# patrikhuber/superviseddescent

Measured on NVIDIA H100. Metric: faces/sec RCR 22-landmark detect, higher is better.
Workload: dtype f32

## Files before the change

superviseddescent_b200/csrc/sd_hog.cu:

```cuda
#include "sd_internal.cuh"
#include "sd_hog_common.cuh"

#include <cmath>
#include <cuda_pipeline.h>

namespace {

constexpr int kHogThreads = 256;

struct HogArgs {
    const uint8_t* images;
    int width, height, row_stride;
    long long image_stride;
    int image_count;
    const int* image_index;
    const sd_roi* roi;
    const sd_frame* frames;
    uint8_t* roi_miss;
    const float* x;
    long long ldx;
    int N, L;
    int variant, nc, cs, K, fs, dd;
    const int* half;
    HogOrient orient;
    const int* rtab;
    const float* btab;
    int tma_count;
    float* A;
    long long ld;
    int* geometry;
    uint8_t* patches;
    int8_t* bins;
    int* status;
};

__global__ void hog_geometry_kernel(const float* __restrict__ x, long long ldx, int N, int L, const sd_eyes_dev eyes, float rel,
                                    int fixed_half, int fs, int* __restrict__ half_out, int* __restrict__ rtab, int* __restrict__ status,
                                    uint8_t* __restrict__ face_flag)
{
    const int i = blockIdx.x;
    if (i >= N) return;
    __shared__ int s_half;
    if (threadIdx.x == 0) {
        bool degenerate;
        const int half = sd_patch_half(x + (long long)i * ldx, L, eyes, rel, fixed_half, &degenerate);
        if (degenerate) {
            atomicOr(status, 1);
            if (face_flag) face_flag[i] = 1;
        }
        half_out[i] = half;
        s_half = half;
    }
    __syncthreads();
    const int P = 2 * s_half;
    int* rt = rtab + (long long)i * 5 * fs;
    for (int t = threadIdx.x; t < fs; t += blockDim.x) {
        const HogResizeTap r = hog_resize_tap(t, fs, P);
        rt[t] = r.sx;
        rt[fs + t] = r.xw;
        rt[2 * fs + t] = r.y0;
        rt[3 * fs + t] = r.y1;
        rt[4 * fs + t] = r.yw;
    }
}

__global__ void hog_bintab_kernel(int fs, int nc, int cs, int pw, float* __restrict__ btab)
{
    __shared__ int s_sbin[256];
    for (int t = threadIdx.x; t < fs; t += blockDim.x) {
        int b;
        float w1, w2;
        hog_spatial_weight(t, cs, &b, &w1, &w2);
        s_sbin[t] = b;
        if (t >= 1 && t <= fs - 2)
            for (int c = 0; c < nc; ++c) btab[c * pw + t - 1] = (b == c) ? w1 : ((b == c - 1) ? w2 : 0.f);
        else if (t == fs - 1 && pw > fs - 2)
            for (int c = 0; c < nc; ++c) btab[c * pw + pw - 1] = 0.f;
    }
    __syncthreads();
    int* lohi = reinterpret_cast<int*>(btab + nc * pw);
    for (int c = threadIdx.x; c < nc; c += blockDim.x) {
        int lo = fs, hi = -1;
        for (int t = 1; t <= fs - 2; ++t) {
            const int b = s_sbin[t];
            if (b == c || b == c - 1) { if (t < lo) lo = t; hi = t; }
        }
        lohi[c] = lo;
        lohi[nc + c] = hi;
    }
}

__device__ __forceinline__ int byte_of(unsigned lo, unsigned hi, int n) { return (int)(((n < 4 ? lo : hi) >> (8 * (n & 3))) & 0xffu); }

struct HogSmem {
    int patch, bin, r1, tab, xa, wcell, lo, hi, vote, mbar, stage_end, total;
    int pp;
    int pb, pm;
    int pw;
    int tpad;
};

__host__ __device__ inline int align_up(int v, int a) { return (v + a - 1) / a * a; }

__host__ __device__ inline HogSmem hog_smem_layout(int fs, int nc, int K)
{
    HogSmem s;
    s.pp = align_up(fs, 4);
    s.pm = align_up(fs - 2, 4) + 1;
    s.pb = s.pm - 1;
    if ((s.pb & 7) == 0 && (fs - 2) * (s.pb + 4) <= fs * fs) s.pb += 4;
    int o = 0;
    s.patch = o;
    o = align_up(s.pp * fs, 16);
    s.tab = o;    o += fs * 16;
    s.xa = o;     o += fs * 4;
    s.pw = align_up(fs - 2, 2);
    s.wcell = align_up(o, 8); o = s.wcell + nc * s.pw * 4;
    s.lo = o;     o += nc * 4;
    s.hi = o;     o += nc * 4;
    s.mbar = align_up(o, 8); o = s.mbar + 8;
    o = align_up(o, 128);
    s.bin = o;    o = align_up(o + fs * fs, 16);
    s.r1 = o;     o = align_up(o + fs * fs * 4, 16);
    s.tpad = align_up((fs - 2) * nc, 32);
    s.vote = o;
    o += 2 * K * s.tpad * 4;
    s.stage_end = o;
    s.total = align_up(o + 8, 16);
    return s;
}

constexpr int kTmaClasses = 8;
__host__ __device__ constexpr int hog_tma_box(int c) { return c == 0 ? 32 : c == 1 ? 48 : c == 2 ? 64 : c == 3 ? 80 : c == 4 ? 96 : c == 5 ? 112 : c == 6 ? 128 : 160; }
struct HogMaps { CUtensorMap m[kTmaClasses]; };

template <bool MIR>
__device__ __forceinline__ bool hog_sample_mirrored(const HogArgs& a, int sample)
{
    return MIR && sd_sample_is_mirrored(a.image_index[sample]);
}

template <int KT, int NCT, int CST, int NT, bool MIR>
__global__ void __launch_bounds__(NT, NCT > 0 ? 2048 / NT : 0) hog_patch_kernel(const __grid_constant__ HogArgs a, const __grid_constant__ HogMaps maps)
{
    static_assert(NT % 32 == 0 && NT >= 64, "hog_patch_kernel needs whole warps and at least 64 threads");
    constexpr int kWarps = NT / 32;
    extern __shared__ __align__(128) unsigned char smem[];
    const int K = KT > 0 ? KT : a.K;
    const int nc = NCT > 0 ? NCT : a.nc;
    const int fs = (NCT > 0 && CST > 0) ? NCT * CST : a.fs;
    const int cells = nc * nc;
    const HogSmem lay = hog_smem_layout(fs, nc, K);
    const int pp = lay.pp, pb = lay.pb, pm = lay.pm, pw = lay.pw;
    uint8_t* s_patch = smem + lay.patch;
    int8_t* s_bin = reinterpret_cast<int8_t*>(smem + lay.bin);
    float* s_gmag = reinterpret_cast<float*>(smem + lay.r1);
    int4* s_tab = reinterpret_cast<int4*>(smem + lay.tab);
    short2* s_xa = reinterpret_cast<short2*>(smem + lay.xa);
    float* s_wcell = reinterpret_cast<float*>(smem + lay.wcell);
    int* s_lo = reinterpret_cast<int*>(smem + lay.lo);
    int* s_hi = reinterpret_cast<int*>(smem + lay.hi);
    float* s_T = reinterpret_cast<float*>(smem + lay.vote);
    uint64_t* s_mbar = reinterpret_cast<uint64_t*>(smem + lay.mbar);

    const int tid = threadIdx.x;
    const int lane = tid & 31, warp = tid >> 5;
    const long long patch_id = blockIdx.x;
    const int sample = (int)(patch_id / a.L);
    const int lm = (int)(patch_id - (long long)sample * a.L);

    const float* __restrict__ row = a.x + (long long)sample * a.ldx;
    const int half = __ldg(a.half + sample);
    const int P = 2 * half;
    const int cx = __float2int_rn(row[lm]);
    const int cy = __float2int_rn(row[lm + a.L]);
    int img_idx = a.image_index ? a.image_index[sample] : sample;
    if (MIR) img_idx = sd_sample_frame_of(img_idx);
    if (img_idx < 0 || img_idx >= a.image_count) {
        img_idx = 0;
        if (tid == 0 && a.status) atomicOr(a.status, 2);
    }
    int W = a.width, H = a.height, rs = a.row_stride;
    const uint8_t* __restrict__ img = a.images + (long long)img_idx * a.image_stride;
    if (a.frames) {
        const sd_frame f = a.frames[img_idx];
        W = f.width; H = f.height; rs = f.row_stride;
        img = a.images + f.offset;
    }
    int rx = 0, ry = 0, rw = W, rh = H;
    if (a.roi) {
        const sd_roi r = a.roi[img_idx];
        rx = r.x; ry = r.y; rw = r.w; rh = r.h; rs = r.row_stride;
        img = a.images + r.offset;
    }
    if (tid == 0 && a.geometry) {
        a.geometry[patch_id * 3 + 0] = cx;
        a.geometry[patch_id * 3 + 1] = cy;
        a.geometry[patch_id * 3 + 2] = half;
    }

    const int x0 = sd_window_x0(cx, half, W, hog_sample_mirrored<MIR>(a, sample)), y0 = cy - half;
    uint8_t* s_stage = smem + lay.bin;
    const int stage_cap = lay.stage_end - lay.bin;
    int tma_box = 0;
    const int tma_shift = x0 & 15;
#pragma unroll
    for (int c = kTmaClasses - 1; c >= 0; --c)
        if (c < a.tma_count && hog_tma_box(c) >= P + tma_shift && hog_tma_box(c) * hog_tma_box(c) <= stage_cap) tma_box = hog_tma_box(c);
    if (tma_box > 0 && tid == 0) {
        int cls = 0;
#pragma unroll
        for (int c = 0; c < kTmaClasses; ++c) if (hog_tma_box(c) == tma_box) cls = c;
        hog_tma_load(s_mbar, s_stage, &maps.m[cls], x0 - tma_shift, y0, img_idx, tma_box * tma_box);
    }

    {
        const int* __restrict__ rt = a.rtab + (long long)sample * 5 * fs;
        for (int t = tid; t < fs; t += NT) {
            const int xa = __ldg(rt + fs + t);
            s_xa[t] = *reinterpret_cast<const short2*>(&xa);
            s_tab[t] = make_int4(__ldg(rt + t), __ldg(rt + 2 * fs + t), __ldg(rt + 3 * fs + t), __ldg(rt + 4 * fs + t));
        }
        for (int i = tid; i < nc * pw; i += NT) s_wcell[i] = __ldg(a.btab + i);
        const int* __restrict__ lohi = reinterpret_cast<const int*>(a.btab + nc * pw);
        if (tid < nc) { s_lo[tid] = __ldg(lohi + tid); s_hi[tid] = __ldg(lohi + nc + tid); }
    }
    {
        const bool resident = x0 >= rx && y0 >= ry && x0 + P <= rx + rw && y0 + P <= ry + rh && x0 >= 0 && y0 >= 0 && x0 + P <= W && y0 + P <= H;
        const uintptr_t align_bits = reinterpret_cast<uintptr_t>(img) | (uintptr_t)rs;
        const bool vec16 = !tma_box && resident && (align_bits & 15) == 0;
        const bool words = !tma_box && resident && (align_bits & 3) == 0;
        const int shiftb = tma_box ? tma_shift : (vec16 ? ((x0 - rx) & 15) : (words ? ((x0 - rx) & 3) : 0));
        const int pitch = tma_box ? tma_box : ((P + 15 + 15) & ~15);
        const bool staged = pitch * P <= stage_cap;
        bool miss = false;
        if (staged) {
            if (tma_box) {
            } else if (vec16) {
                const int nvec = (shiftb + P + 15) >> 4;
                const int gs = nvec <= 8 ? 3 : (nvec <= 16 ? 4 : 5);
                const int lv = lane & ((1 << gs) - 1), lr = lane >> gs, rows_per_pass = 32 >> gs;
                const uint8_t* wrow = img + (long long)(y0 - ry) * rs + (x0 - rx - shiftb);
                for (int r = warp * rows_per_pass + lr; r < P; r += kWarps * rows_per_pass)
#pragma unroll 1
                    for (int v = lv; v < nvec; v += (1 << gs))
                        reinterpret_cast<uint4*>(s_stage + r * pitch)[v] = __ldg(reinterpret_cast<const uint4*>(wrow + (long long)r * rs) + v);
            } else if (words) {
                const int nwords = (shiftb + P + 3) >> 2;
                const uint8_t* wrow = img + (long long)(y0 - ry) * rs + (x0 - rx - shiftb);
                for (int r = warp; r < P; r += kWarps) {
                    const uint32_t* src = reinterpret_cast<const uint32_t*>(wrow + (long long)r * rs);
                    uint32_t* dst = reinterpret_cast<uint32_t*>(s_stage + r * pitch);
#pragma unroll 1
                    for (int w = lane; w < nwords; w += 32) dst[w] = __ldg(src + w);
                }
            } else {
                for (int r = warp; r < P; r += kWarps) {
                    const int iy = y0 + r;
                    const bool rowin = (unsigned)iy < (unsigned)H;
                    const bool rowres = iy >= ry && iy < ry + rh;
                    for (int c = lane; c < P; c += 32) {
                        const int ix = x0 + c;
                        int v = 0;
                        if (rowin && (unsigned)ix < (unsigned)W) {
                            if (rowres && ix >= rx && ix < rx + rw) v = __ldg(img + (long long)(iy - ry) * rs + (ix - rx));
                            else miss = true;
                        }
                        s_stage[r * pitch + c] = (uint8_t)v;
                    }
                }
            }
            __syncthreads();
            if (tma_box) hog_tma_wait(s_mbar);
            if (hog_sample_mirrored<MIR>(a, sample)) {
#pragma unroll 1
                for (int r = warp; r < P; r += kWarps) {
                    uint8_t* q = s_stage + r * pitch + shiftb;
#pragma unroll 1
                    for (int c = lane; c < half; c += 32) {
                        const uint8_t u = q[c], v = q[P - 1 - c];
                        q[c] = v;
                        q[P - 1 - c] = u;
                    }
                }
                __syncthreads();
            }
            if (fs <= 64) {
                const int np = (fs + 1) >> 1, groups = NT / np;
                const int j = tid % np, g = tid / np;
                if (g < groups) {
                    const int dxa = 2 * j, dxb = min(dxa + 1, fs - 1);
                    const int sxa = s_tab[dxa].x, sxb = s_tab[dxb].x;
                    const unsigned xa = *reinterpret_cast<const unsigned*>(s_xa + dxa), xb = *reinterpret_cast<const unsigned*>(s_xa + dxb);
                    const int q = (shiftb + sxa) & ~3;
                    const int oa = shiftb + sxa - q, ob = shiftb + sxb - q;
                    uint8_t* out = s_patch + dxa;
                    if (ob <= 6) {
                        const unsigned sa = oa | (oa + 1) << 4, sb = ob | (ob + 1) << 4;
                        const uint8_t* base = s_stage + q;
#pragma unroll 2
                        for (int dy = g; dy < fs; dy += groups) {
                            const int4 yt = s_tab[dy];
                            const unsigned* r0 = reinterpret_cast<const unsigned*>(base + yt.y * pitch);
                            const unsigned* r1 = reinterpret_cast<const unsigned*>(base + yt.z * pitch);
                            const unsigned a0 = r0[0], a1 = r0[1], b0 = r1[0], b1 = r1[1];
                            const int va = hog_resize_out(yt.w, __dp2a_lo(xa, __byte_perm(a0, a1, sa), 0u), __dp2a_lo(xa, __byte_perm(b0, b1, sa), 0u));
                            const int vb = hog_resize_out(yt.w, __dp2a_lo(xb, __byte_perm(a0, a1, sb), 0u), __dp2a_lo(xb, __byte_perm(b0, b1, sb), 0u));
                            *reinterpret_cast<uint16_t*>(out + dy * pp) = (uint16_t)(va | vb << 8);
                        }
                    } else {
                        const int ax = s_xa[dxa].x, bx = s_xa[dxa].y, cx = s_xa[dxb].x, dx = s_xa[dxb].y;
                        const int sxa1 = min(sxa + 1, P - 1), sxb1 = min(sxb + 1, P - 1);
                        const uint8_t* base = s_stage + shiftb;
                        for (int dy = g; dy < fs; dy += groups) {
                            const int4 yt = s_tab[dy];
                            const uint8_t* r0 = base + yt.y * pitch;
                            const uint8_t* r1 = base + yt.z * pitch;
                            const int va = hog_resize_out(yt.w, (int)r0[sxa] * ax + (int)r0[sxa1] * bx, (int)r1[sxa] * ax + (int)r1[sxa1] * bx);
                            const int vb = hog_resize_out(yt.w, (int)r0[sxb] * cx + (int)r0[sxb1] * dx, (int)r1[sxb] * cx + (int)r1[sxb1] * dx);
                            *reinterpret_cast<uint16_t*>(out + dy * pp) = (uint16_t)(va | vb << 8);
                        }
                    }
                }
            } else {
                for (int dy = warp; dy < fs; dy += kWarps) {
                    const int4 yt = s_tab[dy];
                    const uint8_t* r0 = s_stage + yt.y * pitch + shiftb;
                    const uint8_t* r1 = s_stage + yt.z * pitch + shiftb;
                    for (int dx = lane; dx < fs; dx += 32) {
                        const int sx = s_tab[dx].x;
                        const int sx1 = min(sx + 1, P - 1);
                        const short2 xa = s_xa[dx];
                        const int t0 = (int)r0[sx] * xa.x + (int)r0[sx1] * xa.y;
                        const int t1 = (int)r1[sx] * xa.x + (int)r1[sx1] * xa.y;
                        s_patch[dy * pp + dx] = (uint8_t)hog_resize_out(yt.w, t0, t1);
                    }
                }
            }
        } else {
            const bool mirrored = hog_sample_mirrored<MIR>(a, sample);
            __syncthreads();
            for (int dy = warp; dy < fs; dy += kWarps) {
                const int4 yt = s_tab[dy];
                const int iy0 = y0 + yt.y, iy1 = y0 + yt.z;
                for (int dx = lane; dx < fs; dx += 32) {
                    const int sx = s_tab[dx].x;
                    const short2 xa = s_xa[dx];
                    int p[4];
#pragma unroll
                    for (int q = 0; q < 4; ++q) {
                        const int u = sx + (q & 1);
                        const int ix = mirrored ? x0 + P - 1 - u : x0 + u, iy = (q & 2) ? iy1 : iy0;
                        int v = 0;
                        if ((q & 1) && xa.y == 0) { p[q] = 0; continue; }
                        if ((unsigned)ix < (unsigned)W && (unsigned)iy < (unsigned)H) {
                            if (ix >= rx && ix < rx + rw && iy >= ry && iy < ry + rh) v = __ldg(img + (long long)(iy - ry) * rs + (ix - rx));
                            else miss = true;
                        }
                        p[q] = v;
                    }
                    const int t0 = p[0] * xa.x + p[1] * xa.y;
                    const int t1 = p[2] * xa.x + p[3] * xa.y;
                    s_patch[dy * pp + dx] = (uint8_t)hog_resize_out(yt.w, t0, t1);
                }
            }
        }
        if (miss && a.roi_miss) a.roi_miss[img_idx] = 1;
        if (a.patches) {
            __syncthreads();
            for (int i = tid; i < fs * fs; i += NT) {
                const int y = i / fs;
                a.patches[patch_id * fs * fs + i] = s_patch[y * pp + (i - y * fs)];
            }
        }
    }
    __syncthreads();

    {
        const int iw = fs - 2, runs = (iw + 3) >> 2, nitem = iw * runs;
        const int pw = pp >> 2;
        for (int i = tid; i < nitem; i += NT) {
            const int y = i / runs, r = i - y * runs;
            const unsigned* c = reinterpret_cast<const unsigned*>(s_patch) + (y + 1) * pw + r;
            const unsigned c0 = c[0], c1 = c[1], u0 = c[-pw], u1 = c[1 - pw], d0 = c[pw], d1 = c[pw + 1];
            unsigned bins = 0;
            float* gm = s_gmag + y * pm + 4 * r;
#pragma unroll
            for (int k = 0; k < 4; ++k) {
                const int gx = byte_of(c0, c1, k + 2) - byte_of(c0, c1, k);
                const int gy = byte_of(d0, d1, k + 1) - byte_of(u0, u1, k + 1);
                const int g2 = gx * gx + gy * gy;
                const float g = __fsqrt_rn((float)g2);
                const int b = hog_bin(a.orient, K, gx, gy, g);
                bins |= (unsigned)(b & 0xff) << (8 * k);
                gm[k] = b < 0 ? 0.f : g;
            }
            *reinterpret_cast<unsigned*>(s_bin + y * pb + 4 * r) = bins;
        }
    }
    if (a.bins) {
        __syncthreads();
        for (int idx = tid; idx < fs * fs; idx += NT) {
            const int y = idx / fs, x = idx - y * fs;
            const bool interior = x >= 1 && x <= fs - 2 && y >= 1 && y <= fs - 2;
            a.bins[patch_id * fs * fs + idx] = interior ? s_bin[(y - 1) * pb + x - 1] : (int8_t)-1;
        }
    }
    if (!a.A) return;
    __syncthreads();

    {
        const int nrow = fs - 2, ntask = nrow * nc, tpad = lay.tpad;
        for (int task = tid; task < ntask; task += NT) {
            const int ci = task / nrow, y = 1 + task - ci * nrow;
            const int xlo = s_lo[ci], xhi = s_hi[ci];
            const int8_t* bp = s_bin + (y - 1) * pb - 1;
            const float* gp = s_gmag + (y - 1) * pm - 1;
            const float* wp = s_wcell + ci * pw - 1;
            float* T = s_T + task;
            for (int b = 0; b < 2 * K; ++b) T[b * tpad] = 0.f;
            const auto vote = [&](int b, float p) { float* q = T + max(b, 0) * tpad; *q = __fadd_rn(*q, p); };
            int x = xlo;
            if (!(x & 1) && x <= xhi) { vote(bp[x], __fmul_rn(gp[x], wp[x])); ++x; }
#pragma unroll 1
            for (; x < xhi; x += 2) {
                const unsigned bb = *reinterpret_cast<const unsigned short*>(bp + x);
                const float2 w = *reinterpret_cast<const float2*>(wp + x);
                vote((int)(int8_t)bb, __fmul_rn(gp[x], w.x));
                vote((int)(int8_t)(bb >> 8), __fmul_rn(gp[x + 1], w.y));
            }
            if (x == xhi) vote(bp[x], __fmul_rn(gp[x], wp[x]));
        }
        __syncthreads();
        float* __restrict__ out = a.A + (long long)sample * a.ld + (long long)lm * cells * a.dd;
        for (int i = tid; i < K * cells; i += NT) {
            const int b = i / cells, c = i - b * cells;
            const int cj = c / nc, ci = c - cj * nc;
            const int ylo = s_lo[cj], yhi = s_hi[cj];
            const float* Tp = s_T + b * tpad + ci * nrow + (ylo - 1);
            const float* wy = s_wcell + cj * pw + (ylo - 1);
            float acc = 0.f, acc2 = 0.f;
#pragma unroll 1
            for (int y = ylo; y <= yhi; ++y) {
                const float w = *wy++;
                acc = __fadd_rn(acc, __fmul_rn(Tp[0], w));
                acc2 = __fadd_rn(acc2, __fmul_rn(Tp[K * tpad], w));
                ++Tp;
            }
            out[i] = acc;
            out[i + K * cells] = acc2;
        }
    }
}

struct NormArgs {
    float* A;
    long long ld;
    int N, L, nc, K, dd, variant, per_cta;
};

__host__ __device__ inline int hog_norm_smem(int nc, int K, int per_cta)
{
    const int cells = nc * nc;
    return per_cta * (8 + 2 * K * cells * 4 + cells * 8 + (nc + 1) * (nc + 1) * 8);
}

template <int KT>
__global__ void __launch_bounds__(kHogThreads) hog_normalise_kernel(const NormArgs a)
{
    extern __shared__ __align__(16) unsigned char s_norm[];
    const int K = KT > 0 ? KT : a.K;
    const int nc = a.nc, nb = nc + 1, cells = nc * nc, blocks = nb * nb, hsz = 2 * K * cells, per_lm = cells * a.dd;
    const long long first = (long long)blockIdx.x * a.per_cta;
    const int np = (int)min((long long)a.per_cta, (long long)a.N * a.L - first);
    long long* s_slice = reinterpret_cast<long long*>(s_norm);
    double* s_energy = reinterpret_cast<double*>(s_slice + a.per_cta);
    double* s_fac = s_energy + a.per_cta * cells;
    float* s_hist = reinterpret_cast<float*>(s_fac + a.per_cta * blocks);
    for (int p = threadIdx.x; p < np; p += kHogThreads) {
        const long long id = first + p;
        const int sample = (int)(id / a.L), lm = (int)(id - (long long)sample * a.L);
        s_slice[p] = (long long)sample * a.ld + (long long)lm * per_lm;
        if (lm == 0) a.A[(long long)sample * a.ld + (long long)a.L * per_lm] = 1.0f;
    }
    __syncthreads();
    for (int i = threadIdx.x; i < np * hsz; i += kHogThreads) {
        const int p = i / hsz;
        __pipeline_memcpy_async(s_hist + i, a.A + s_slice[p] + (i - p * hsz), sizeof(float));
    }
    __pipeline_commit();
    __pipeline_wait_prior(0);
    __syncthreads();
    for (int i = threadIdx.x; i < np * cells; i += kHogThreads) {
        const int p = i / cells, c = i - p * cells;
        s_energy[i] = (double)hog_cell_energy(s_hist + p * hsz + c, cells, K);
    }
    __syncthreads();
    for (int i = threadIdx.x; i < np * blocks; i += kHogThreads) {
        const int p = i / blocks, j = i - p * blocks;
        const int jy = j / nb, jx = j - jy * nb;
        s_fac[i] = hog_block_factor(s_energy + p * cells, nc, max(jx - 1, 0), min(jx, nc - 1), max(jy - 1, 0), min(jy, nc - 1));
    }
    __syncthreads();
    for (int i = threadIdx.x; i < np * cells; i += kHogThreads) {
        const int p = i / cells, c = i - p * cells;
        const int cj = c / nc, ci = c - cj * nc;
        const double* F = s_fac + p * blocks + cj * nb + ci;
        const double fac[4] = {F[0], F[1], F[nb], F[nb + 1]};
        float* __restrict__ out = a.A + s_slice[p] + ci * nc + cj;
        hog_cell_features(fac, s_hist + p * hsz + c, cells, K, a.variant, [=](int d, float v) { out[d * cells] = v; });
    }
}

template <bool MIR>
decltype(&hog_patch_kernel<0, 0, 0, kHogThreads, MIR>) pick_hog_kernel(int K, int nc, int cs, int* threads)
{
    *threads = kHogThreads;
    if (nc == 5 && (K == 4 || K == 9)) {
#define SD_HOG_PICK(KK, CC, TT) if (K == KK && cs == CC) { *threads = TT; return hog_patch_kernel<KK, 5, CC, TT, MIR>; }
        SD_HOG_PICK(4, 11, 224) SD_HOG_PICK(4, 10, 160) SD_HOG_PICK(4, 8, 160) SD_HOG_PICK(4, 6, 128)
        SD_HOG_PICK(9, 11, 256) SD_HOG_PICK(9, 10, 160) SD_HOG_PICK(9, 8, 160) SD_HOG_PICK(9, 6, 128)
#undef SD_HOG_PICK
    }
    return K == 4 ? hog_patch_kernel<4, 0, 0, kHogThreads, MIR> : K == 9 ? hog_patch_kernel<9, 0, 0, kHogThreads, MIR>
                                                                       : hog_patch_kernel<0, 0, 0, kHogThreads, MIR>;
}

int launch_hog(sd_ctx* ctx, const sd_image_batch* images, const int32_t* d_image_index, bool mirrors, const float* d_x,
               int64_t ldx, int N, int L, const sd_normalisation* eyes, const sd_hog_param* p, float* d_A,
               int64_t ld, int32_t* d_geometry, uint8_t* d_patches, int8_t* d_bins, uint8_t* d_face_degenerate = nullptr)
{
    SD_REQUIRE(ctx, images && images->d_data && d_x && p, "null argument");
    SD_REQUIRE(ctx, N >= 0 && L >= 1, "bad sample / landmark count");
    if (const int rc = sd_hog_check_config(ctx, __func__, p->variant, p->num_bins)) return rc;
    SD_REQUIRE(ctx, p->num_cells >= 1 && p->cell_size >= 1, "bad cell configuration");
    const int fs = p->num_cells * p->cell_size;
    SD_REQUIRE(ctx, fs > 3 && fs <= 256, "resized patch must be 4..256 px (hog.c:545-546 asserts > 3)");
    SD_REQUIRE(ctx, (fs + p->cell_size / 2) / p->cell_size == p->num_cells, "hogWidth != num_cells");
    SD_REQUIRE(ctx, ldx >= 2 * L, "ldx < 2L");
    if (N == 0) return SD_OK;
    const bool fixed = !eyes || eyes->kind == 0;
    int fixed_half = 0;
    if (fixed) {
        fixed_half = p->num_cells * (p->cell_size / 2);
        SD_REQUIRE(ctx, 2 * fixed_half == fs, "the fixed-patch HogTransform needs an even cell_size (patch == num_cells * cell_size)");
    } else if (eyes->kind != 1) {
        return sd_fail(ctx, SD_ERR_INVALID, "unknown normalisation kind");
    }

    HogArgs a;
    sd_eyes_dev eyes_dev;
    memset(&eyes_dev, 0, sizeof(eyes_dev));
    int rc = fixed ? SD_OK : sd_eyes_to_dev(ctx, eyes, L, &eyes_dev);
    if (rc) return rc;
    a.images = images->d_data;
    a.width = images->width; a.height = images->height; a.row_stride = images->row_stride;
    a.image_stride = images->image_stride; a.image_count = images->count;
    a.image_index = d_image_index;
    a.roi = images->d_roi;
    a.roi_miss = images->d_roi_miss;
    a.frames = images->d_frames;
    if (!d_image_index) SD_REQUIRE(ctx, images->count >= N, "fewer images than samples and no image index");
    a.x = d_x; a.ldx = ldx; a.N = N; a.L = L;
    a.variant = p->variant; a.nc = p->num_cells; a.cs = p->cell_size; a.K = p->num_bins; a.fs = fs;
    a.dd = sd_hog_dd(p->num_bins, p->variant);
    a.A = d_A; a.ld = ld;
    if (d_A) SD_REQUIRE(ctx, ld >= (int64_t)L * a.nc * a.nc * a.dd + 1, "ld < feature length");
    const HogSmem lay = hog_smem_layout(fs, a.nc, a.K);
    const int cells = a.nc * a.nc;
    NormArgs na;
    na.A = d_A; na.ld = ld; na.N = N; na.L = L; na.nc = a.nc; na.K = a.K; na.dd = a.dd; na.variant = a.variant;
    na.per_cta = cells < kHogThreads ? kHogThreads / cells : 1;
    const int norm_smem = hog_norm_smem(a.nc, a.K, na.per_cta);
    SD_REQUIRE(ctx, lay.total <= 227 * 1024 && norm_smem <= 227 * 1024, "HOG configuration needs more than 227 KB of shared memory");
    const long long blocks = (long long)N * L;
    SD_REQUIRE(ctx, blocks < 2147483647LL, "too many patches for one launch");
    a.geometry = d_geometry; a.patches = d_patches; a.bins = d_bins;
    a.status = reinterpret_cast<int*>(ctx->d_scratch) + 1;

    hog_orientations(a.K, a.orient);

    const size_t geom_bytes = (size_t)N * sizeof(int) + (size_t)N * 5 * fs * sizeof(int) + (size_t)(a.nc * fs + 2 * a.nc) * sizeof(float);
    int* d_half = (int*)sd_workspace(ctx, SD_WS_GEOM, geom_bytes);
    if (!d_half) return SD_ERR_CUDA;
    int* d_rtab = d_half + N;
    float* d_btab = reinterpret_cast<float*>(d_rtab + (size_t)N * 5 * fs);
    hog_geometry_kernel<<<N, 64, 0, ctx->stream>>>(d_x, ldx, N, L, eyes_dev, p->relative_patch_size, fixed_half, fs, d_half, d_rtab, a.status,
                                                    d_face_degenerate);
    SD_LAUNCH_CHECK(ctx, "hog_geometry_kernel");
    hog_bintab_kernel<<<1, 256, 0, ctx->stream>>>(fs, a.nc, a.cs, lay.pw, d_btab);
    SD_LAUNCH_CHECK(ctx, "hog_bintab_kernel");
    a.half = d_half;
    a.rtab = d_rtab;
    a.btab = d_btab;

    HogMaps maps;
    memset(&maps, 0, sizeof(maps));
    a.tma_count = 0;
    if (!images->d_roi && (images->image_stride % 16) == 0 && (images->count == 1 || images->image_stride > 0)) {
        for (int c = 0; c < kTmaClasses && hog_tma_box(c) <= 256; ++c) {
            if (!hog_frame_map(images, hog_tma_box(c), hog_tma_box(c), &maps.m[c])) break;
            a.tma_count = c + 1;
        }
    }

    int threads = kHogThreads;
    const auto kern = mirrors && d_image_index ? pick_hog_kernel<true>(a.K, a.nc, a.cs, &threads)
                                               : pick_hog_kernel<false>(a.K, a.nc, a.cs, &threads);
    SD_CUDA(ctx, cudaFuncSetAttribute(kern, cudaFuncAttributeMaxDynamicSharedMemorySize, lay.total));
    kern<<<(unsigned)blocks, threads, lay.total, ctx->stream>>>(a, maps);
    SD_LAUNCH_CHECK(ctx, "hog_patch_kernel");
    if (!d_A) return SD_OK;
    auto norm = a.K == 4 ? hog_normalise_kernel<4> : a.K == 9 ? hog_normalise_kernel<9> : hog_normalise_kernel<0>;
    SD_CUDA(ctx, cudaFuncSetAttribute(norm, cudaFuncAttributeMaxDynamicSharedMemorySize, norm_smem));
    norm<<<(unsigned)sd_div_up(blocks, na.per_cta), kHogThreads, norm_smem, ctx->stream>>>(na);
    SD_LAUNCH_CHECK(ctx, "hog_normalise_kernel");
    return SD_OK;
}

}

int sd_hog_batch_unmirrored(sd_ctx* ctx, const sd_image_batch* images, const int32_t* d_image_index, const float* d_x, int64_t ldx,
                            int num_samples, int num_landmarks, const sd_normalisation* eyes, const sd_hog_param* p, float* d_A,
                            int64_t ld, uint8_t* d_face_degenerate)
{
    if (num_samples == 0) return SD_OK;
    SD_REQUIRE(ctx, d_A, "null output");
    return launch_hog(ctx, images, d_image_index, false, d_x, ldx, num_samples, num_landmarks, eyes, p, d_A, ld, nullptr, nullptr,
                      nullptr, d_face_degenerate);
}

namespace {
__global__ void bgr2gray_kernel(const uint8_t* __restrict__ bgr, int width, int height, long long srow, long long simg, int count,
                                uint8_t* __restrict__ gray, long long drow, long long dimg, int vec_ok)
{
    const int groups = (width + 3) >> 2;
    const long long total = (long long)count * height * groups;
    for (long long t = blockIdx.x * (long long)blockDim.x + threadIdx.x; t < total; t += (long long)gridDim.x * blockDim.x) {
        const int g = (int)(t % groups);
        const long long ry = t / groups;
        const int y = (int)(ry % height);
        const long long im = ry / height;
        const uint8_t* s = bgr + im * simg + (long long)y * srow + 12 * g;
        uint8_t* d = gray + im * dimg + (long long)y * drow + 4 * g;
        const int x0 = 4 * g;
        if (vec_ok && x0 + 4 <= width) {
            const uint32_t w0 = *reinterpret_cast<const uint32_t*>(s), w1 = *reinterpret_cast<const uint32_t*>(s + 4),
                           w2 = *reinterpret_cast<const uint32_t*>(s + 8);
            const uint32_t b0 = w0 & 255, g0 = (w0 >> 8) & 255, r0 = (w0 >> 16) & 255, b1 = w0 >> 24;
            const uint32_t g1 = w1 & 255, r1 = (w1 >> 8) & 255, b2 = (w1 >> 16) & 255, g2 = w1 >> 24;
            const uint32_t r2 = w2 & 255, b3 = (w2 >> 8) & 255, g3 = (w2 >> 16) & 255, r3 = w2 >> 24;
            const uint32_t y0 = sd_bgr_to_gray(b0, g0, r0), y1 = sd_bgr_to_gray(b1, g1, r1);
            const uint32_t y2 = sd_bgr_to_gray(b2, g2, r2), y3 = sd_bgr_to_gray(b3, g3, r3);
            *reinterpret_cast<uint32_t*>(d) = y0 | (y1 << 8) | (y2 << 16) | (y3 << 24);
        } else {
            for (int k = 0; k < 4 && x0 + k < width; ++k) d[k] = (uint8_t)sd_bgr_to_gray(s[3 * k], s[3 * k + 1], s[3 * k + 2]);
        }
    }
}
}

extern "C" {

int sd_hog_feature_length(int num_landmarks, const sd_hog_param* p)
{
    if (!p) return -1;
    const int dd = sd_hog_dd(p->num_bins, p->variant);
    return num_landmarks * p->num_cells * p->num_cells * dd + 1;
}

int sd_hog_batch(sd_ctx* ctx, const sd_image_batch* images, const int32_t* d_image_index, const float* d_x,
                 int64_t ldx, int num_samples, int num_landmarks, const sd_normalisation* eyes,
                 const sd_hog_param* p, float* d_A, int64_t ld)
{
    if (!ctx) return SD_ERR_INVALID;
    if (num_samples == 0) return SD_OK;
    SD_REQUIRE(ctx, d_A, "null output");
    return launch_hog(ctx, images, d_image_index, true, d_x, ldx, num_samples, num_landmarks, eyes, p, d_A, ld,
                      nullptr, nullptr, nullptr);
}

int sd_hog_debug(sd_ctx* ctx, const sd_image_batch* images, const int32_t* d_image_index, const float* d_x,
                 int64_t ldx, int num_samples, int num_landmarks, const sd_normalisation* eyes,
                 const sd_hog_param* p, int32_t* d_geometry, uint8_t* d_patches, int8_t* d_bins)
{
    if (!ctx) return SD_ERR_INVALID;
    return launch_hog(ctx, images, d_image_index, true, d_x, ldx, num_samples, num_landmarks, eyes, p, nullptr, 0,
                      d_geometry, d_patches, d_bins);
}

int sd_bgr2gray(sd_ctx* ctx, const uint8_t* d_bgr, int width, int height, int64_t bgr_row_stride, int64_t bgr_image_stride,
                int count, uint8_t* d_gray, int64_t gray_row_stride, int64_t gray_image_stride)
{
    if (!ctx) return SD_ERR_INVALID;
    SD_REQUIRE(ctx, count >= 0 && width > 0 && height > 0, "bad argument");
    if (count == 0) return SD_OK;
    SD_REQUIRE(ctx, d_bgr && d_gray && bgr_row_stride >= 3LL * width && gray_row_stride >= width, "bad argument");
    const int vec_ok = ((reinterpret_cast<uintptr_t>(d_bgr) | reinterpret_cast<uintptr_t>(d_gray) | (uintptr_t)bgr_row_stride |
                         (uintptr_t)bgr_image_stride | (uintptr_t)gray_row_stride | (uintptr_t)gray_image_stride) & 3) == 0;
    const long long total = (long long)count * height * ((width + 3) >> 2);
    const int blocks = (int)(sd_div_up(total, 256) < 16LL * ctx->sm_count ? sd_div_up(total, 256) : 16LL * ctx->sm_count);
    bgr2gray_kernel<<<blocks, 256, 0, ctx->stream>>>(d_bgr, width, height, bgr_row_stride, bgr_image_stride, count, d_gray,
                                                     gray_row_stride, gray_image_stride, vec_ok);
    SD_LAUNCH_CHECK(ctx, "bgr2gray_kernel");
    return SD_OK;
}

}
```

Measured before the change: 839,100.

## Make HOG normalise kernel persistent with double-buffered vectorised async loads

The HOG block-normalisation kernel becomes a persistent grid sized from occupancy. Each CTA loops over patch groups and double-buffers histogram loads in shared memory, so the next group's cp.async copies overlap the current group's energy, factor and feature computation. Loads are issued per warp with 16-byte async copies when the layout is aligned. The kernel is also templated on the cell count, and the bias-column write moves into the output loop. The cost is twice the shared memory per CTA, which can lower occupancy, plus more register pressure.

Result: no change. 854,000 (median of 6 runs) (+1.8%).

```diff
diff --git a/superviseddescent_b200/csrc/sd_hog.cu b/superviseddescent_b200/csrc/sd_hog.cu
--- a/superviseddescent_b200/csrc/sd_hog.cu
+++ b/superviseddescent_b200/csrc/sd_hog.cu
@@ -456,59 +456,81 @@
 struct NormArgs {
     float* A;
     long long ld;
-    int N, L, nc, K, dd, variant, per_cta;
+    int N, L, nc, K, dd, variant, per_cta, vec;
 };
 
+__host__ __device__ constexpr int hog_norm_pitch(int nc, int K) { return (2 * K * nc * nc + 3) & ~3; }
+
+__host__ __device__ constexpr int hog_norm_per_cta(int cells) { return cells < kHogThreads ? kHogThreads / cells : 1; }
+
 __host__ __device__ inline int hog_norm_smem(int nc, int K, int per_cta)
 {
-    const int cells = nc * nc;
-    return per_cta * (8 + 2 * K * cells * 4 + cells * 8 + (nc + 1) * (nc + 1) * 8);
-}
-
-template <int KT>
+    return per_cta * (2 * hog_norm_pitch(nc, K) * 4 + nc * nc * 8 + (nc + 1) * (nc + 1) * 8);
+}
+
+template <int KT, int NCT>
 __global__ void __launch_bounds__(kHogThreads) hog_normalise_kernel(const NormArgs a)
 {
     extern __shared__ __align__(16) unsigned char s_norm[];
     const int K = KT > 0 ? KT : a.K;
-    const int nc = a.nc, nb = nc + 1, cells = nc * nc, blocks = nb * nb, hsz = 2 * K * cells, per_lm = cells * a.dd;
-    const long long first = (long long)blockIdx.x * a.per_cta;
-    const int np = (int)min((long long)a.per_cta, (long long)a.N * a.L - first);
-    long long* s_slice = reinterpret_cast<long long*>(s_norm);
-    double* s_energy = reinterpret_cast<double*>(s_slice + a.per_cta);
-    double* s_fac = s_energy + a.per_cta * cells;
-    float* s_hist = reinterpret_cast<float*>(s_fac + a.per_cta * blocks);
-    for (int p = threadIdx.x; p < np; p += kHogThreads) {
-        const long long id = first + p;
-        const int sample = (int)(id / a.L), lm = (int)(id - (long long)sample * a.L);
-        s_slice[p] = (long long)sample * a.ld + (long long)lm * per_lm;
-        if (lm == 0) a.A[(long long)sample * a.ld + (long long)a.L * per_lm] = 1.0f;
-    }
-    __syncthreads();
-    for (int i = threadIdx.x; i < np * hsz; i += kHogThreads) {
-        const int p = i / hsz;
-        __pipeline_memcpy_async(s_hist + i, a.A + s_slice[p] + (i - p * hsz), sizeof(float));
-    }
-    __pipeline_commit();
-    __pipeline_wait_prior(0);
-    __syncthreads();
-    for (int i = threadIdx.x; i < np * cells; i += kHogThreads) {
-        const int p = i / cells, c = i - p * cells;
-        s_energy[i] = (double)hog_cell_energy(s_hist + p * hsz + c, cells, K);
-    }
-    __syncthreads();
-    for (int i = threadIdx.x; i < np * blocks; i += kHogThreads) {
-        const int p = i / blocks, j = i - p * blocks;
-        const int jy = j / nb, jx = j - jy * nb;
-        s_fac[i] = hog_block_factor(s_energy + p * cells, nc, max(jx - 1, 0), min(jx, nc - 1), max(jy - 1, 0), min(jy, nc - 1));
-    }
-    __syncthreads();
-    for (int i = threadIdx.x; i < np * cells; i += kHogThreads) {
-        const int p = i / cells, c = i - p * cells;
-        const int cj = c / nc, ci = c - cj * nc;
-        const double* F = s_fac + p * blocks + cj * nb + ci;
-        const double fac[4] = {F[0], F[1], F[nb], F[nb + 1]};
-        float* __restrict__ out = a.A + s_slice[p] + ci * nc + cj;
-        hog_cell_features(fac, s_hist + p * hsz + c, cells, K, a.variant, [=](int d, float v) { out[d * cells] = v; });
+    const int nc = NCT > 0 ? NCT : a.nc, nb = nc + 1, cells = nc * nc, blocks = nb * nb, hsz = 2 * K * cells, per_lm = cells * a.dd;
+    const int per_cta = NCT > 0 ? hog_norm_per_cta(NCT * NCT) : a.per_cta;
+    const int hp = hog_norm_pitch(nc, K), buf_floats = per_cta * hp;
+    const int patches = a.N * a.L;
+    const int groups = (patches + per_cta - 1) / per_cta;
+    float* s_hist = reinterpret_cast<float*>(s_norm);
+    double* s_energy = reinterpret_cast<double*>(s_hist + 2 * buf_floats);
+    double* s_fac = s_energy + per_cta * cells;
+    const int warp = threadIdx.x >> 5, lane = threadIdx.x & 31;
+    const auto slice = [&](int id) {
+        const int sample = id / a.L, lm = id - sample * a.L;
+        return (long long)sample * a.ld + (long long)lm * per_lm;
+    };
+    const auto stage = [&](int g, float* dst) {
+        if (g < groups) {
+            const int first = g * per_cta, np = min(per_cta, patches - first);
+            for (int p = warp; p < np; p += kHogThreads / 32) {
+                const float* src = a.A + slice(first + p);
+                float* d = dst + p * hp;
+                if (a.vec)
+                    for (int j = 4 * lane; j < hsz; j += 128) __pipeline_memcpy_async(d + j, src + j, 16);
+                else
+                    for (int j = lane; j < hsz; j += 32) __pipeline_memcpy_async(d + j, src + j, sizeof(float));
+            }
+        }
+        __pipeline_commit();
+    };
+    int buf = 0;
+    stage(blockIdx.x, s_hist);
+    for (int g = blockIdx.x; g < groups; g += gridDim.x, buf ^= 1) {
+        stage(g < groups - (int)gridDim.x ? g + (int)gridDim.x : groups, s_hist + (buf ^ 1) * buf_floats);
+        __pipeline_wait_prior(1);
+        __syncthreads();
+        const float* hist = s_hist + buf * buf_floats;
+        const int first = g * per_cta, np = min(per_cta, patches - first);
+        for (int i = threadIdx.x; i < np * cells; i += kHogThreads) {
+            const int p = i / cells, c = i - p * cells;
+            s_energy[i] = (double)hog_cell_energy(hist + p * hp + c, cells, K);
+        }
+        __syncthreads();
+        for (int i = threadIdx.x; i < np * blocks; i += kHogThreads) {
+            const int p = i / blocks, j = i - p * blocks;
+            const int jy = j / nb, jx = j - jy * nb;
+            s_fac[i] = hog_block_factor(s_energy + p * cells, nc, max(jx - 1, 0), min(jx, nc - 1), max(jy - 1, 0), min(jy, nc - 1));
+        }
+        __syncthreads();
+        for (int i = threadIdx.x; i < np * cells; i += kHogThreads) {
+            const int p = i / cells, c = i - p * cells;
+            const int cj = c / nc, ci = c - cj * nc;
+            const double* F = s_fac + p * blocks + cj * nb + ci;
+            const double fac[4] = {F[0], F[1], F[nb], F[nb + 1]};
+            const int id = first + p, sample = id / a.L;
+            float* __restrict__ row = a.A + (long long)sample * a.ld;
+            float* __restrict__ out = row + (long long)(id - sample * a.L) * per_lm + ci * nc + cj;
+            hog_cell_features(fac, hist + p * hp + c, cells, K, a.variant, [=](int d, float v) { out[d * cells] = v; });
+            if (c == 0 && id == sample * a.L) row[(long long)a.L * per_lm] = 1.0f;
+        }
+        __syncthreads();
     }
 }
 
@@ -570,7 +592,8 @@
     const int cells = a.nc * a.nc;
     NormArgs na;
     na.A = d_A; na.ld = ld; na.N = N; na.L = L; na.nc = a.nc; na.K = a.K; na.dd = a.dd; na.variant = a.variant;
-    na.per_cta = cells < kHogThreads ? kHogThreads / cells : 1;
+    na.per_cta = hog_norm_per_cta(cells);
+    na.vec = (ld % 4) == 0 && ((long long)cells * a.dd) % 4 == 0 && (reinterpret_cast<uintptr_t>(d_A) & 15) == 0;
     const int norm_smem = hog_norm_smem(a.nc, a.K, na.per_cta);
     SD_REQUIRE(ctx, lay.total <= 227 * 1024 && norm_smem <= 227 * 1024, "HOG configuration needs more than 227 KB of shared memory");
     const long long blocks = (long long)N * L;
@@ -611,9 +634,13 @@
     kern<<<(unsigned)blocks, threads, lay.total, ctx->stream>>>(a, maps);
     SD_LAUNCH_CHECK(ctx, "hog_patch_kernel");
     if (!d_A) return SD_OK;
-    auto norm = a.K == 4 ? hog_normalise_kernel<4> : a.K == 9 ? hog_normalise_kernel<9> : hog_normalise_kernel<0>;
+    auto norm = a.nc == 5 && a.K == 4 ? hog_normalise_kernel<4, 5> : a.nc == 5 && a.K == 9 ? hog_normalise_kernel<9, 5>
+              : a.K == 4 ? hog_normalise_kernel<4, 0> : a.K == 9 ? hog_normalise_kernel<9, 0> : hog_normalise_kernel<0, 0>;
     SD_CUDA(ctx, cudaFuncSetAttribute(norm, cudaFuncAttributeMaxDynamicSharedMemorySize, norm_smem));
-    norm<<<(unsigned)sd_div_up(blocks, na.per_cta), kHogThreads, norm_smem, ctx->stream>>>(na);
+    int norm_per_sm = 0;
+    SD_CUDA(ctx, cudaOccupancyMaxActiveBlocksPerMultiprocessor(&norm_per_sm, norm, kHogThreads, norm_smem));
+    const long long groups = sd_div_up(blocks, na.per_cta);
+    norm<<<(unsigned)std::min(groups, (long long)std::max(norm_per_sm, 1) * ctx->sm_count), kHogThreads, norm_smem, ctx->stream>>>(na);
     SD_LAUNCH_CHECK(ctx, "hog_normalise_kernel");
     return SD_OK;
 }
```
